# kekeliu-whu/Wildcat-SLAM

Hardware: AMD Instinct MI355X
Metric: surfel-extract Mpts/s (higher is better)
Workload: dtype f64; 1 GPU; C2: 1M-pt single scan (G2 patch lattice, 999936 pts -> 31248 surfels) per GPU, voxel-grid + 3-level octree + per-cell 3x3 PCA; input = the reference's 48-byte hilti_ros::Point records, consumed in place; points_per_gpu=999936, surfels_per_gpu=31248, parallelism=sweep-per-gpu x1

## Files before the change

wildcat-slam_amd/csrc/ctx.h:

```cpp
#pragma once
#include <hip/hip_runtime.h>

#include <cstdarg>
#include <cstdio>
#include <cstdlib>
#include <cstring>
#include <string>
#include <vector>

#include "../../include/wildcat_hip.h"

struct wc_window_state;

struct wc_buf {
  void *p = nullptr;
  size_t cap = 0;
  bool pooled = false;
  bool plain = false;
};

#ifdef WC_DEV_KNOBS
#define WC_DBG(P, bit) ((P).dbg & (bit))
#else
#define WC_DBG(P, bit) 0
#endif

struct wc_dev_opts {
  int exact_sums = 0;
  int debug_skip = 0;
  int fx_merge_min = 3;
  int fx_split = -1;
  int no_bucket_sort = 0;
  int ex_sync = 0;
  int match_pair_serial = 0;
  int lm_dense = 0;
  int lm_side_stream = 1;
  int lm_one_collective = 0;
  int lm_dense_radius = 7;
  int lm_radius0 = -1;
};
inline bool wc_log_env(const char *name) { return getenv(name) != nullptr; }

struct wc_ctx {
  int device = 0;
  wc_params P;
  wc_dev_opts dev;
  bool pool_ok = false;
  hipMemPool_t pool = nullptr;
  hipStream_t own_stream = nullptr;
  hipStream_t stream = nullptr;
  hipEvent_t ev0 = nullptr, ev1 = nullptr;
  std::string err;
  wc_buf b_ex_ctrl;
  wc_buf b_keys[2], b_vals[2], b_sorttmp, b_slots, b_slot_ids, b_slot_keys[2], b_slot_idx[2], b_cand, b_cand_meta,
      b_status, b_misc[8], b_route[4], b_fx[10];
  double match_stats[8] = {0, 0, 0, 0, 0, 0, 0, 0};
  wc_buf b_kd[10];
  std::vector<wc_ctx *> batch_subs;
  wc_buf b_batch;
  wc_buf b_match_half;
  hipEvent_t ev_knn[2] = {nullptr, nullptr};
  wc_comm comm{};
  bool have_comm = false;
  void *rccl = nullptr;
  uint32_t *h_status_dev = nullptr;
  uint32_t *h_status = nullptr;
  unsigned long long mail_ticket = 0;
  wc_buf b_stage;
  void *h_stage = nullptr;
  size_t h_stage_cap = 0;
  double *h_mail = nullptr;
  struct {
    bool active = false;
    wc_points pts;
    double t_lo, t_hi;
    wc_surfel *d_out;
    wc_surfel_id *d_ids;
    uint64_t cap;
    bool wide;
    bool general;
    bool order_general = false;
    int general_calls = 0;
    bool bucket_attr_set = false;
    uint32_t lds_cap = 256;
// ... 101 lines not shown
```

wildcat-slam_amd/csrc/ctx.hip:

```cpp
#include "ctx.h"

#include <cmath>
#include <cstring>
#include <mutex>

extern "C" const char *wc_version(void) { return "wildcat_hip 0.1 (gfx950)"; }

extern "C" int wc_device_count(void) {
  int n = 0;
  if (hipGetDeviceCount(&n) != hipSuccess) return 0;
  return n;
}

extern "C" void wc_params_default(wc_params *p) {
  std::memset(p, 0, sizeof(*p));
  p->voxel_size = 0.8f;
  p->max_layer = 2;
  p->min_points = 20;
  p->planer_threshold = 0.01f;
  p->min_plane_likeness = 0.1;
  p->cluster_gap = 0.05;
  p->cluster_min_points = 20;
  p->center_scale = 1.0;
  p->angular_scale = 5.0 * M_PI / 180.0;
  p->surfel_dist_max = 0.1;
  p->knn_k = 10;
  p->time_diff_min = 0.06;
  p->surfel_sigma0 = 0.05 / 6;
  p->cauchy_a = 0.4;
  const double gn = 0.00015198973532354657, an = 0.006308226052016165;
  const double gw = 0.00011673723527962174, aw = 2.664506559330434e-06;
  const double rate = 200, k = 0.01;
  p->w_gyr = 1 / (gn * std::sqrt(rate)) * k;
  p->w_acc = 1 / (an * std::sqrt(rate)) * k;
  p->w_bg = 1 / (gw / std::sqrt(rate)) * k;
  p->w_ba = 1 / (aw / std::sqrt(rate)) * k;
  p->imu_dt = 1 / rate;
  p->max_iterations = 100;
  p->reference_quirks = 1;
  p->exact_sums = 0;
}

static int check_params(wc_ctx *ctx, const wc_params *p) {
  if (p->max_layer < 0 || p->max_layer > 2) return wc_fail(ctx, WC_ERR_ARG, "max_layer must be 0..2");
  if (!(p->voxel_size > 0)) return wc_fail(ctx, WC_ERR_ARG, "voxel_size must be positive");
  if (p->cluster_min_points < 1 || p->min_points < 0) return wc_fail(ctx, WC_ERR_ARG, "bad point thresholds");
  if (p->knn_k < 1 || p->knn_k > 16) return wc_fail(ctx, WC_ERR_ARG, "knn_k must be 1..16");
  return WC_OK;
}

namespace {
struct DevOpt {
  const char *name, *env;
  int wc_dev_opts::*field;
  bool flag_only;
};
const DevOpt kDevOpts[] = {
    {"exact_sums", "WC_EXACT_SUMS", &wc_dev_opts::exact_sums, true},
    {"debug_skip", "WC_DEBUG_SKIP", &wc_dev_opts::debug_skip, false},
    {"fx_merge_min", "WC_FX_MERGE_MIN", &wc_dev_opts::fx_merge_min, false},
    {"fx_split", "WC_FX_SPLIT", &wc_dev_opts::fx_split, false},
    {"no_bucket_sort", "WC_NO_BUCKET_SORT", &wc_dev_opts::no_bucket_sort, true},
    {"ex_sync", "WC_EX_SYNC", &wc_dev_opts::ex_sync, true},
    {"match_pair_serial", "WC_MATCH_PAIR_SERIAL", &wc_dev_opts::match_pair_serial, true},
    {"lm_dense", "WC_LM_DENSE", &wc_dev_opts::lm_dense, true},
    {"lm_one_collective", "WC_LM_ONE_COLLECTIVE", &wc_dev_opts::lm_one_collective, true},
    {"lm_side_stream", "WC_LM_SIDE_STREAM", &wc_dev_opts::lm_side_stream, false},
    {"lm_dense_radius", "WC_LM_DENSE_RADIUS", &wc_dev_opts::lm_dense_radius, false},
    {"lm_radius0", "WC_LM_RADIUS0", &wc_dev_opts::lm_radius0, false},
};
}

namespace {
struct DevPool {
  hipMemPool_t pool = nullptr;
  int refs = 0;
};
std::mutex g_pool_mu;
DevPool g_pools[64];
}
hipMemPool_t wc_pool_acquire(int device) {
  if (device < 0 || device >= 64) return nullptr;
  std::lock_guard<std::mutex> lk(g_pool_mu);
  DevPool &d = g_pools[device];
  if (!d.pool) {
    int supported = 0;
    if (hipDeviceGetAttribute(&supported, hipDeviceAttributeMemoryPoolsSupported, device) != hipSuccess || !supported) {
      (void)hipGetLastError();
      return nullptr;
    }
    hipMemPoolProps props;
    std::memset(&props, 0, sizeof(props));
    props.allocType = hipMemAllocationTypePinned;
    props.handleTypes = hipMemHandleTypeNone;
    props.location.type = hipMemLocationTypeDevice;
    props.location.id = device;
    hipMemPool_t p = nullptr;
    if (hipMemPoolCreate(&p, &props) != hipSuccess || !p) {
      (void)hipGetLastError();
      return nullptr;
    }
    uint64_t keep = ~0ull;
    if (hipMemPoolSetAttribute(p, hipMemPoolAttrReleaseThreshold, &keep) != hipSuccess) (void)hipGetLastError();
    d.pool = p;
  }
  ++d.refs;
  return d.pool;
}
void wc_pool_release(int device, hipMemPool_t pool) {
  if (!pool || device < 0 || device >= 64) return;
  std::lock_guard<std::mutex> lk(g_pool_mu);
  DevPool &d = g_pools[device];
  if (d.pool == pool && --d.refs == 0) {
    (void)hipMemPoolDestroy(d.pool);
// ... 278 lines not shown
```

wildcat-slam_amd/csrc/extract.hip:

```cpp
#include <hip/hip_runtime.h>
#include <type_traits>

#include <chrono>
#include <cstdlib>
#include <cstring>
#include <rocprim/rocprim.hpp>

#include "ctx.h"
#include "dmath.h"

namespace {

constexpr int kMom = 11;
constexpr int kProdStride = 66;
constexpr unsigned kRootsGrid = 256 * 16;
constexpr unsigned kEmitGrid = 256 * 8;
constexpr unsigned kRoots2Grid = 256 * 4;
constexpr int kBuckets = 4096;
constexpr int kTile = 2048;
constexpr uint32_t kFlagKeyRange = 1u, kFlagSlotOverflow = 2u, kFlagTimeRange = 4u, kFlagBucketOverflow = 8u, kFlagSlotBinOverflow = 16u, kFlagLdsOverflow = 32u;

struct ExParams {
  double vs;
  float vs_f;
// ... 1511 lines not shown
    if (i < nb) {
      s_off[i] = carry + inc - l;
      bin[i] = c;
      run_off[(size_t)b * bin_cap + i] = carry + inc - l;
    }
    carry += __shfl(inc, 63);
  }
  __builtin_amdgcn_wave_barrier();
  uint32_t *s_list = (uint32_t *)s_a;
  uint32_t nlive = 0, next_head = nb;
  for (int i0 = (int)((nb + 63) / 64) * 64 - 64; i0 >= 0; i0 -= 64) {
    const uint32_t r = (uint32_t)i0 + lane;
    const bool in = r < nb;
    const uint32_t rest = in ? comp_rest(s_b[r]) : 0u;
    const bool head = in && (r == 0 || comp_rest(s_b[r - 1]) != rest);
    const unsigned long long hm = __ballot(head);
    const unsigned long long above = (lane == 63) ? 0ull : (hm >> (lane + 1));
    const uint32_t r2 = above ? r + (uint32_t)__ffsll((long long)above) : next_head;
    const uint32_t seg = (r2 < nb ? s_off[min(r2, nb - 1)] : total) - (in ? s_off[r] : 0u);
    const bool live = head && seg > (uint32_t)min_points;
    const unsigned long long lm = __ballot(live);
    if (live) s_list[nlive + (uint32_t)__popcll(lm & ((1ull << lane) - 1ull))] = r | (r2 << 16);
    nlive += (uint32_t)__popcll(lm);
    if (hm) next_head = (uint32_t)i0 + (uint32_t)__ffsll((long long)hm) - 1u;
  }
  if (lane == 0) s_live[w] = nlive;
  __syncthreads();
  const uint32_t pbase0 = s_red[0] + s_red[1] + s_red[2] + s_red[3];
  const uint32_t pbase = pbase0 + before;
  const uint32_t first_slot = pbase0 / (uint32_t)(min_points + 1);
  uint32_t lbase = 0;
  for (int j = 0; j < w; ++j) lbase += s_live[j];
  if (t == 0) {
    root_cnt[blockIdx.x] = s_live[0] + s_live[1] + s_live[2] + s_live[3];
    root_first[blockIdx.x] = first_slot;
  }
  for (uint32_t k = lane; k < nlive; k += 64) {
    const uint32_t r = s_list[k] & 0xFFFFu, r2 = s_list[k] >> 16;
    const uint32_t seg = (r2 < nb ? s_off[r2] : total) - s_off[r];
    head_slots[first_slot + lbase + k] = HeadRec{pbase + s_off[r], b * bin_cap + r, r2 - r, seg};
  }
}

constexpr uint32_t kPtBinMax = 1024;

inline uint32_t pt_bin_cap(uint64_t n) {
  uint32_t cap = 64;
  while (cap < kPtBinMax && (uint64_t)cap * kBuckets < 32 * n) cap *= 2;
  return cap;
}

constexpr uint32_t kCtrlStatus = 0, kCtrlCounts = 64, kCtrlRoots = kCtrlCounts + 2 * kBuckets, kCtrlBins = kCtrlRoots + 2 * (kBuckets / 4),
                   kCtrlFx = kCtrlBins + kBuckets, kCtrlWords = kCtrlFx + 4 * 16 * 32;

int clear_ctrl(wc_ctx *ctx) {
  WC_TRY(wc_ensure(ctx, ctx->b_ex_ctrl, kCtrlWords * 4));
  uint32_t *ctrl = (uint32_t *)ctx->b_ex_ctrl.p;
  InitArgs I{};
  void *dp = nullptr;
  if (hipHostGetDevicePointer(&dp, ctx->h_status, 0) != hipSuccess) dp = nullptr;
  const unsigned long long a = (unsigned long long)dp;
  I.p[0] = ctrl, I.nw[0] = 8, I.val[0] = 0u;
  I.p[1] = ctrl + 10, I.nw[1] = kCtrlRoots - 10, I.val[1] = 0u;
  I.p[2] = ctrl + 8, I.nw[2] = 1, I.val[2] = (uint32_t)a;
  I.p[3] = ctrl + 9, I.nw[3] = 1, I.val[3] = (uint32_t)(a >> 32);
  I.p[4] = ctrl + kCtrlBins, I.nw[4] = kBuckets + 4 * 16 * 32, I.val[4] = 0u;
  k_init<<<(kCtrlRoots + 255) / 256, 256, 0, ctx->stream>>>(I);
  WC_HIP(ctx, hipGetLastError());
  return WC_OK;
}

int point_sort_runs(wc_ctx *ctx, const wc_points &pts, double vs, HeadRec *head_slots, int min_points, uint32_t *status) {
  hipStream_t st = ctx->stream;
  const uint64_t n = pts.n;
  const uint32_t cap = pt_bin_cap(n);
  const uint32_t lds_cap = std::min(cap, std::max(64u, ctx->ex.lds_cap));
  WC_TRY(wc_ensure(ctx, ctx->b_misc[1], (uint64_t)kBuckets * cap * 8));
  WC_TRY(wc_ensure(ctx, ctx->b_misc[3], (uint64_t)kBuckets * cap * 4));
  uint32_t *counts = (uint32_t *)ctx->b_ex_ctrl.p + kCtrlCounts;
  const unsigned tiles = (unsigned)((n + kTile - 1) / kTile);
  const size_t lds = (size_t)4 * lds_cap * 20;
  if (!ctx->ex.bucket_attr_set) {
    WC_HIP(ctx, hipFuncSetAttribute((const void *)k_pt_bucket, hipFuncAttributeMaxDynamicSharedMemorySize, (int)(4 * kPtBinMax * 20)));
    ctx->ex.bucket_attr_set = true;
  }
  k_pt_runs<<<tiles, kRunThreads, 0, st>>>(pts, vs, n, counts, (uint64_t *)ctx->b_misc[1].p, cap, status);
  k_pt_bucket<<<kBuckets / 4, 256, lds, st>>>((uint64_t *)ctx->b_misc[1].p, cap, lds_cap, counts, (uint32_t *)ctx->b_misc[3].p, head_slots,
                                             counts + 2 * kBuckets, counts + 2 * kBuckets + kBuckets / 4, min_points, status);
  WC_HIP(ctx, hipGetLastError());
  return WC_OK;
}

template <typename K>
int sort_pairs(wc_ctx *ctx, K *kin, K *kout, uint32_t *vin, uint32_t *vout, size_t n, unsigned end_bit) {
  using cfg = rocprim::radix_sort_config<rocprim::default_config, rocprim::default_config, rocprim::default_config, 0>;
  size_t tmp = 0;
  WC_HIP(ctx, rocprim::radix_sort_pairs<cfg>(nullptr, tmp, kin, kout, vin, vout, n, 0u, end_bit, ctx->stream));
  WC_TRY(wc_ensure(ctx, ctx->b_sorttmp, tmp));
  tmp = ctx->b_sorttmp.cap;
  WC_HIP(ctx, rocprim::radix_sort_pairs<cfg>(ctx->b_sorttmp.p, tmp, kin, kout, vin, vout, n, 0u, end_bit, ctx->stream));
  return WC_OK;
}

#include "extract_fast.inc"
#include "extract_split.inc"

int fx_ensure_zero(wc_ctx *ctx, wc_buf &b, size_t bytes) {
  if (bytes <= b.cap) return WC_OK;
  WC_TRY(wc_ensure(ctx, b, bytes));
  WC_HIP(ctx, hipMemsetAsync(b.p, 0, b.cap, ctx->stream));
  return WC_OK;
}

bool fx_applicable(const wc_ctx *ctx, uint64_t n, double t_lo, double t_hi) {
  const wc_params &P = ctx->P;
  if (P.exact_sums || ctx->dev.exact_sums) return false;
  if (n < 64 || !(P.voxel_size > 0.0f) || P.voxel_size >= 0.99f) return false;
  if (!(P.cluster_gap > 1e-6) || !(t_hi > t_lo)) return false;
  if ((t_hi - t_lo) / (P.cluster_gap * 0.999) >= 1048000.0) return false;
  return true;
}

int fx_tail(wc_ctx *ctx, bool layer2);

int run_pipeline_fast(wc_ctx *ctx, const wc_points &pts, double t_lo, double t_hi, wc_surfel *d_out, wc_surfel_id *d_ids, uint64_t cap) {
  const wc_params &P = ctx->P;
  const uint64_t n = pts.n;
  hipStream_t st = ctx->stream;
  FxArgs A;
  std::memset(&A, 0, sizeof(A));
  ExParams &E = A.P;
  E.vs = (double)P.voxel_size, E.vs_f = P.voxel_size, E.max_layer = P.max_layer, E.min_points = P.min_points;
  E.thr = (double)P.planer_threshold, E.min_like = P.min_plane_likeness;
  for (int i = 0; i < 3; ++i) E.view[i] = P.view_point[i];
  E.gap = P.cluster_gap, E.cluster_min = P.cluster_min_points;
  E.t_lo_bits = ordered_bits_host(t_lo);
  E.t_span_bits = ordered_bits_host(t_hi) - E.t_lo_bits;
  E.dbg = ctx->dev.debug_skip;
  E.merge_min = ctx->dev.fx_merge_min;
  unsigned tbits = 1;
  while (tbits < 64 && (E.t_span_bits >> tbits)) ++tbits;
  A.pts = pts;
  A.t_lo = t_lo;
  int e = 0;
  (void)std::frexp(t_hi - t_lo, &e);
  A.tick = std::ldexp(1.0, 40 - e), A.inv_tick = std::ldexp(1.0, e - 40);
  A.inv_w = 1.0 / (P.cluster_gap * 0.999);
  A.inv_span = 1.0 / (t_hi - t_lo);
  A.inv_vs = 1.0 / (double)P.voxel_size;
  A.qs = 4294967296.0, A.inv_q = 1.0 / 4294967296.0, A.inv_qq = std::ldexp(1.0, -44);
  uint32_t mr = 1024;
  while ((uint64_t)mr * 8 < n) mr *= 2;
  A.mr_per = mr / kFxSub, A.mq_per = std::max(64u, mr / 2 / kFxSub);
  uint32_t tr = 2048;
  while ((uint64_t)tr * 4 < n) tr *= 2;
  A.tr_mask = tr - 1;
  A.static_map = n <= 2000000ull ? 1u : 0u;
  {
    const uintptr_t px = (uintptr_t)pts.xyz, pt = (uintptr_t)pts.time;
    if (pts.xyz_stride == 48u && pts.time_stride == 48u && pt == px + 24u && px % 16u == 0u)
      A.fmt = 1u;
    else if (pts.xyz_stride == 12u && pts.time_stride == 8u && px % 16u == 0u && pt % 16u == 0u)
      A.fmt = 2u;
  }
  const unsigned tiles = (unsigned)((n + kFxTile - 1) / kFxTile);
  A.rec_tiles = tiles;
  const uint64_t spill_full = ((uint64_t)tiles + 7) / 8 * kFxTile;
  A.spill_per = (uint32_t)((n <= 8000000ull || ctx->ex.fx_spill_full) ? spill_full : std::max<uint64_t>(1024, n / 32));
  A.rec_cap = tiles * (uint32_t)kFxRecTile + 8u * A.spill_per;
  const uint64_t total_slots = std::max<uint64_t>((n * (uint64_t)(P.max_layer + 1)) / (uint64_t)P.cluster_min_points + 1, (uint64_t)kFxSub * 256);
  uint32_t bin_cap = 64;
  while (bin_cap < kSlotBinMax && (uint64_t)bin_cap * kBuckets < 2 * total_slots) bin_cap *= 2;
  WC_TRY(fx_ensure_zero(ctx, ctx->b_fx[0], (size_t)tr * 4));
  WC_TRY(wc_ensure(ctx, ctx->b_fx[1], (size_t)mr * 4));
  WC_TRY(fx_ensure_zero(ctx, ctx->b_fx[2], (size_t)tr * kFxBlockW * 8));
  WC_TRY(fx_ensure_zero(ctx, ctx->b_fx[3], (size_t)A.mq_per * kFxSub * kFxBlockW * 8));
  WC_TRY(wc_ensure(ctx, ctx->b_fx[4], (size_t)2 * A.rec_cap * kFxRecW * 8));
  const unsigned ngrid = std::min<unsigned>(256 * 16, std::max<unsigned>(64, (unsigned)(n / 256)));
  WC_TRY(wc_ensure(ctx, ctx->b_fx[6], (size_t)ngrid * kFxJobCap * kFxJobW * 8));
  ctx->ex.fx_split = ctx->ex.batch_defer || (ctx->dev.fx_split >= 0 ? ctx->dev.fx_split != 0 : !A.static_map);
  if (ctx->ex.fx_split) {
    A.static_map = 0u;
    A.jobpool_per = (uint32_t)std::max<uint64_t>(4096, n / (uint64_t)std::max(1, P.cluster_min_points) / 2);
    WC_TRY(wc_ensure(ctx, ctx->b_fx[7], ((size_t)mr / 8 + 2) * kFxNodeW * 64 * 8));
    WC_TRY(wc_ensure(ctx, ctx->b_fx[8], ((size_t)mr / 8 + 2) * kFxDescW * 4));
    WC_TRY(wc_ensure(ctx, ctx->b_fx[9], (size_t)8 * A.jobpool_per * kFxJobW * 8));
    A.nodes = (unsigned long long *)ctx->b_fx[7].p, A.wdesc = (uint32_t *)ctx->b_fx[8].p, A.jobpool = (unsigned long long *)ctx->b_fx[9].p;
  }
  WC_TRY(wc_ensure(ctx, ctx->b_slots, total_slots * sizeof(wc_surfel)));
  WC_TRY(wc_ensure(ctx, ctx->b_slot_ids, total_slots * sizeof(wc_surfel_id)));
  WC_TRY(wc_ensure(ctx, ctx->b_slot_keys[1], (uint64_t)kBuckets * bin_cap * 8));
  if (ctx->ex.fx_dirty) {
    for (int i : {0, 2, 3}) WC_HIP(ctx, hipMemsetAsync(ctx->b_fx[i].p, 0, ctx->b_fx[i].cap, st));
    ctx->ex.fx_dirty = false;
  }
  WC_TRY(wc_ensure(ctx, ctx->b_fx[5], (size_t)2 * kCtrlWords * 4));
  if (!ctx->ex.fx_ctrl_ready) {
    WC_HIP(ctx, hipMemsetAsync(ctx->b_fx[5].p, 0, (size_t)2 * kCtrlWords * 4, st));
    void *dp = nullptr;
    if (hipHostGetDevicePointer(&dp, ctx->h_status, 0) != hipSuccess) dp = nullptr;
    const unsigned long long a = (unsigned long long)dp;
    const uint32_t addr[2] = {(uint32_t)a, (uint32_t)(a >> 32)};
    for (int b = 0; b < 2; ++b)
      WC_HIP(ctx, hipMemcpyAsync((uint32_t *)ctx->b_fx[5].p + (size_t)b * kCtrlWords + 8, addr, 8, hipMemcpyHostToDevice, st));
    WC_HIP(ctx, hipStreamSynchronize(st));
    ctx->ex.fx_ctrl_ready = true;
    ctx->ex.fx_parity = 0;
  }
  uint32_t *ctrl = (uint32_t *)ctx->b_fx[5].p + (size_t)ctx->ex.fx_parity * kCtrlWords;
  for (int q = 0; q < 64; ++q) ctx->h_status[q] = 0;
// ... 651 lines not shown
```

wildcat-slam_amd/csrc/extract_fast.inc:

```

constexpr uint32_t kFlagFxFallback = 64u;
constexpr int kFxPts = 4;
constexpr int kFxThreads = 256;
constexpr int kFxTile = kFxPts * kFxThreads;
constexpr int kFxLds = 256;
constexpr int kFxLdsProbe = 12;
constexpr int kFxDirect = 16;
constexpr int kFxRecTile = kFxLds + (kFxThreads / 64) * 4 * kFxDirect;
constexpr int kFxSlots = 16;
constexpr int kFxRecW = 16;
constexpr int kFxHdrW = 16;
constexpr int kFxBlockW = kFxHdrW + 8 * kFxSlots / 2;
constexpr int kFxSub = 16;
constexpr uint32_t kFxStRoots = 0, kFxStNodes2 = 1, kFxStSlots = 2, kFxStSpillBank = 3;
constexpr int kFxCntStride = 32;
constexpr int kFxCntWords = 4 * kFxSub * kFxCntStride;
constexpr unsigned long long kFxTMax = 0xFFFFFFFFFFFFull;
constexpr double kFxMagic = 6755399441055744.0, kFxMagic2 = 7083549724304467820544.0;
constexpr unsigned long long kFxMagicBits = 0x4338000000000000ull;
constexpr uint32_t kFxMagicHi = 0x43380000u, kFxMagic2Hi = 0x44780000u;

struct FxArgs {
  wc_points pts;
  ExParams P;
  double t_lo;
  double tick, inv_tick;
  double inv_w;
  double inv_span;
  double inv_vs;
  double qs, inv_q, inv_qq;
  uint32_t *rkey;
  uint32_t *rlist;
  uint32_t tr_mask;
  uint32_t static_map;
  unsigned long long *blk;
  unsigned long long *blk2;
  unsigned long long *rec;
  uint32_t rec_tiles;
  uint32_t spill_per;
  uint32_t rec_cap;
  uint32_t mr_per, mq_per;
  uint32_t fmt;
  uint32_t *status;
  uint32_t *cnt;
  unsigned long long *jobs;
  unsigned long long *nodes;
  uint32_t *wdesc;
  unsigned long long *jobpool;
  uint32_t jobpool_per;
  wc_surfel *slots;
  wc_surfel_id *slot_ids;
  uint32_t slots_per;
  uint32_t *slot_counts;
  uint64_t *slot_bins;
  uint32_t slot_bin_cap;
};

__device__ __forceinline__ void fx_fallback(uint32_t *status, int why) {
  raise_flag(status, kFlagFxFallback);
  uint32_t *hm = host_mailbox(status);
  if (hm) hm[32 + why] = 1u;
}
__device__ __forceinline__ uint32_t *fx_cnt(const FxArgs &A, uint32_t bank, uint32_t j) { return A.cnt + (bank * kFxSub + j) * kFxCntStride; }

__device__ __forceinline__ uint32_t fx_hash32(uint32_t k) {
  k ^= k >> 16;
  k *= 0x7FEB352Du;
  k ^= k >> 15;
  k *= 0x846CA68Bu;
  k ^= k >> 16;
  return k;
}

__device__ __forceinline__ int fx_vox(double p, double vs, double inv_vs) {
  const double q = p * inv_vs;
  const double r = rint(q);
  if (fabs(q - r) > 1e-9 * (fabs(r) + 1.0)) return (int)floor(q);
  return (int)floor(p / vs);
}

constexpr int kFxStMaxProbe = 20;
__device__ __forceinline__ uint32_t fx_root_slot(const FxArgs &A, uint32_t key1, uint32_t sub, bool insert, uint32_t maxprobe = 0u) {
  uint32_t slot = fx_hash32(key1) & A.tr_mask;
  for (int probe = 0; probe < 64; ++probe) {
    uint32_t k;
    if (insert) {
      k = atomicCAS(&A.rkey[slot], 0u, key1);
      if (k == 0u) {
        if (probe) atomicMax(&A.status[kFxStMaxProbe], (uint32_t)probe);
        const uint32_t local = atomicAdd(fx_cnt(A, kFxStRoots, sub), 1u);
        if (local < A.mr_per)
          A.rlist[sub * A.mr_per + local] = slot;
        else
          fx_fallback(A.status, 0);
        return slot;
      }
    } else {
      k = __hip_atomic_load(&A.rkey[slot], __ATOMIC_RELAXED, __HIP_MEMORY_SCOPE_AGENT);
      if (k == 0u && (uint32_t)probe >= maxprobe) return 0xFFFFFFFFu;
    }
    if (k == key1) return slot;
    slot = (slot + 1u) & A.tr_mask;
  }
  fx_fallback(A.status, 1);
  return 0xFFFFFFFFu;
}

struct FxPart {
  uint32_t n;
  long long st, s[3], ss[6];
  unsigned long long tmin_inv, tmax_p1;
};
__device__ __forceinline__ void fx_zero(FxPart &a) {
  a.n = 0, a.st = 0, a.tmin_inv = 0, a.tmax_p1 = 0;
  for (int i = 0; i < 3; ++i) a.s[i] = 0;
  for (int i = 0; i < 6; ++i) a.ss[i] = 0;
}
__device__ __forceinline__ void fx_acc(FxPart &a, const FxPart &b) {
  a.n += b.n, a.st += b.st;
  for (int i = 0; i < 3; ++i) a.s[i] += b.s[i];
  for (int i = 0; i < 6; ++i) a.ss[i] += b.ss[i];
  a.tmin_inv = max(a.tmin_inv, b.tmin_inv);
  a.tmax_p1 = max(a.tmax_p1, b.tmax_p1);
}

__device__ __forceinline__ void fx_add_cell(unsigned long long *cell, const FxPart &a) {
  atomicAdd((uint32_t *)cell, a.n);
  atomicAdd(&cell[1], (unsigned long long)a.st);
  for (int i = 0; i < 3; ++i) atomicAdd(&cell[2 + i], (unsigned long long)a.s[i]);
  for (int i = 0; i < 6; ++i) atomicAdd(&cell[5 + i], (unsigned long long)a.ss[i]);
  atomicMax(&cell[11], a.tmin_inv);
  atomicMax(&cell[12], a.tmax_p1);
}

struct FxEarly {
  uint32_t key1, s0, found;
  int lead;
};
template <int LEVEL>
__device__ __forceinline__ void fx_push(const FxArgs &A, bool active, unsigned long long code, const FxPart &a, uint32_t sub, uint32_t ridx,
                                        const FxEarly &E) {
  const int lane = threadIdx.x & 63;
  unsigned long long *blk = nullptr;
  uint32_t oct, bin, pkey;
  if (LEVEL == 1) {
    pkey = (uint32_t)(code & 0x3FFFFFFFull) + 1u;
    oct = (uint32_t)(code >> 30) & 7u;
    bin = (uint32_t)(code >> 33) & 0xFFFFFu;
  } else {
    pkey = (uint32_t)(code & 0xFFFFFFFull) + 1u;
    oct = (uint32_t)(code >> 28) & 7u;
    bin = (uint32_t)(code >> 31) & 0xFFFFFu;
  }
  int lead = lane;
  uint32_t gmb = bin;
  {
    unsigned long long todo = __ballot(active);
    while (todo) {
      const int first = __ffsll((long long)todo) - 1;
      const uint32_t k0 = (uint32_t)__shfl((int)pkey, first);
      const bool mine = active && pkey == k0;
      uint32_t mb = mine ? bin : 0xFFFFFFFFu;
      for (int m = 1; m < 64; m <<= 1) mb = min(mb, (uint32_t)__shfl_xor((int)mb, m));
      if (mine) lead = first, gmb = mb;
      todo &= ~__ballot(mine);
    }
  }
  const bool leader = active && lane == lead;
  uint32_t slot = 0xFFFFFFFFu;
  bool created = false;
  const uint32_t e_found = (uint32_t)__shfl((int)E.found, E.lead);
  const bool e_have = LEVEL == 1 && E.key1 != 0u && E.key1 == pkey;
  if (leader) {
    if (LEVEL == 1) {
      if (WC_DBG(A.P, 64)) {
        slot = fx_hash32(pkey) & A.tr_mask;
      } else {
        uint32_t s = fx_hash32(pkey) & A.tr_mask;
        int probe = 0;
        if (e_have) {
          if (e_found == 0u || e_found == pkey) {
            slot = s;
          } else {
            s = (s + 1u) & A.tr_mask;
            probe = 1;
          }
        }
        for (; slot == 0xFFFFFFFFu && probe < 64; ++probe) {
          const uint32_t k = atomicCAS(&A.rkey[s], 0u, pkey);
          if (k == 0u || k == pkey) {
            slot = s;
            created = k == 0u;
            if (created && probe) atomicMax(&A.status[kFxStMaxProbe], (uint32_t)probe);
            break;
          }
          s = (s + 1u) & A.tr_mask;
        }
        if (slot == 0xFFFFFFFFu) fx_fallback(A.status, 2);
      }
    } else {
      slot = pkey - 1u;
    }
  }
  const unsigned long long cm = __ballot(created);
  uint32_t list_base = 0;
  const int cfirst = cm ? __ffsll((long long)cm) - 1 : 0;
  if (cm && lane == cfirst) list_base = atomicAdd(fx_cnt(A, kFxStRoots, sub), (uint32_t)__popcll(cm));
  if (leader && slot != 0xFFFFFFFFu && !(WC_DBG(A.P, 8))) {
    unsigned long long *b0 = (LEVEL == 1 ? A.blk : A.blk2) + (size_t)slot * kFxBlockW;
    atomicMax((uint32_t *)b0 + 2, 0xFFFFFFFFu - gmb);
  }
  const uint32_t myslot = (uint32_t)__shfl((int)slot, lead);
  uint32_t old = 0;
  const bool ok = active && myslot != 0xFFFFFFFFu;
  if (ok) {
    blk = (LEVEL == 1 ? A.blk : A.blk2) + (size_t)myslot * kFxBlockW;
    uint32_t *heads = (uint32_t *)(blk + kFxHdrW);
    if (!(WC_DBG(A.P, 32))) old = atomicExch(&heads[oct * kFxSlots + (bin & (kFxSlots - 1))], ridx + 1u);
  }
  if (cm) {
    list_base = (uint32_t)__shfl((int)list_base, cfirst);
    if (created) {
      const uint32_t local = list_base + (uint32_t)__popcll(cm & ((1ull << lane) - 1ull));
      if (local < A.mr_per)
        A.rlist[sub * A.mr_per + local] = slot;
      else
        fx_fallback(A.status, 3);
    }
  }
  if (!ok) return;
  if (WC_DBG(A.P, 16)) return;
  unsigned long long *rec = A.rec + ((size_t)(LEVEL - 1) * A.rec_cap + ridx) * kFxRecW;
  ulonglong2 *r2 = (ulonglong2 *)rec;
  r2[0] = make_ulonglong2((unsigned long long)a.n | ((unsigned long long)bin << 32), (unsigned long long)a.st);
  r2[1] = make_ulonglong2((unsigned long long)a.s[0], (unsigned long long)a.s[1]);
  r2[2] = make_ulonglong2((unsigned long long)a.s[2], (unsigned long long)a.ss[0]);
  r2[3] = make_ulonglong2((unsigned long long)a.ss[1], (unsigned long long)a.ss[2]);
  r2[4] = make_ulonglong2((unsigned long long)a.ss[3], (unsigned long long)a.ss[4]);
  r2[5] = make_ulonglong2((unsigned long long)a.ss[5], a.tmin_inv);
  r2[6] = make_ulonglong2(a.tmax_p1, (unsigned long long)old);
}

struct FxRaw {
  float x[kFxPts], y[kFxPts], z[kFxPts];
  double t[kFxPts];
};
__device__ __forceinline__ FxRaw fx_acc_load(const FxArgs &A, const uint32_t bid) {
  FxRaw r;
  const uint64_t tb = (uint64_t)bid * kFxTile, n = A.pts.n;
#pragma unroll
  for (int it = 0; it < kFxPts; ++it) {
    const uint64_t i = tb + (uint64_t)it * kFxThreads + threadIdx.x;
    r.x[it] = r.y[it] = r.z[it] = 0.f, r.t[it] = 0.0;
    if (i < n) {
      const float *f = (const float *)((const char *)A.pts.xyz + i * A.pts.xyz_stride);
      r.x[it] = f[0], r.y[it] = f[1], r.z[it] = f[2];
      r.t[it] = load_t(A.pts, i);
    }
  }
  return r;
}

template <int LEVEL>
__device__ __forceinline__ void fx_acc_body(const FxArgs &A, const uint32_t bid) {
  __shared__ unsigned long long lds_raw[kFxLds * 14];
  unsigned long long *h_key = lds_raw;
  unsigned long long(*h_rec)[13] = (unsigned long long(*)[13])(lds_raw + kFxLds);
  static_assert(kFxLds * 14 * 8 >= kFxTile * 20, "staging area fits the hash area");
  const int tid = threadIdx.x;
  const ExParams &P = A.P;
  const uint32_t sub = bid & (kFxSub - 1);
  const uint64_t n = A.pts.n;
  const uint64_t base = ((uint64_t)bid * kFxThreads + tid) * kFxPts;
  static_assert(kFxPts == 4, "the LDS transposition reads four points per lane");
  const bool direct = A.fmt == 2u && ((uint64_t)bid + 1u) * kFxTile <= n;
  FxRaw raw;
  float4 da = make_float4(0.f, 0.f, 0.f, 0.f), db = da, dc = da;
  double2 dt01 = make_double2(0.0, 0.0), dt23 = dt01;
  if (direct) {
    const float4 *xp = (const float4 *)((const char *)A.pts.xyz + base * 12u);
    const double2 *tp = (const double2 *)((const char *)A.pts.time + base * 8u);
    da = xp[0], db = xp[1], dc = xp[2];
    dt01 = tp[0], dt23 = tp[1];
  } else {
    raw = fx_acc_load(A, bid);
  }
  double x0, y0, z0;
  load_xyz(A.pts, 0, x0, y0, z0);
  const int k0x = fx_vox(x0, P.vs, A.inv_vs), k0y = fx_vox(y0, P.vs, A.inv_vs), k0z = fx_vox(z0, P.vs, A.inv_vs);
  const float q0 = P.vs_f / 4;

  double px[kFxPts], py[kFxPts], pz[kFxPts], pt[kFxPts];
  if (direct) {
    const float4 a = da, b = db, c = dc;
    const double2 t01 = dt01, t23 = dt23;
    for (int i = tid; i < kFxLds * 14; i += kFxThreads) lds_raw[i] = 0ull;
    px[0] = a.x, py[0] = a.y, pz[0] = a.z, px[1] = a.w, py[1] = b.x, pz[1] = b.y;
    px[2] = b.z, py[2] = b.w, pz[2] = c.x, px[3] = c.y, py[3] = c.z, pz[3] = c.w;
    pt[0] = t01.x, pt[1] = t01.y, pt[2] = t23.x, pt[3] = t23.y;
    __syncthreads();
  } else {
    double *s_t = (double *)lds_raw;
    float *s_x = (float *)(s_t + kFxTile), *s_y = s_x + kFxTile, *s_z = s_y + kFxTile;
#pragma unroll
    for (int it = 0; it < kFxPts; ++it) {
      s_x[it * kFxThreads + tid] = raw.x[it], s_y[it * kFxThreads + tid] = raw.y[it], s_z[it * kFxThreads + tid] = raw.z[it];
      s_t[it * kFxThreads + tid] = raw.t[it];
    }
    __syncthreads();
    {
      const float4 vx = ((const float4 *)s_x)[tid], vy = ((const float4 *)s_y)[tid], vz = ((const float4 *)s_z)[tid];
      const double2 t01 = ((const double2 *)s_t)[2 * tid], t23 = ((const double2 *)s_t)[2 * tid + 1];
      px[0] = vx.x, px[1] = vx.y, px[2] = vx.z, px[3] = vx.w;
      py[0] = vy.x, py[1] = vy.y, py[2] = vy.z, py[3] = vy.w;
      pz[0] = vz.x, pz[1] = vz.y, pz[2] = vz.z, pz[3] = vz.w;
      pt[0] = t01.x, pt[1] = t01.y, pt[2] = t23.x, pt[3] = t23.y;
    }
    __syncthreads();
    for (int i = tid; i < kFxLds * 14; i += kFxThreads) lds_raw[i] = 0ull;
    __syncthreads();
  }
  if (WC_DBG(P, 4)) {
    double sacc = 0;
#pragma unroll
    for (int j = 0; j < kFxPts; ++j) sacc += px[j] + py[j] + pz[j] + pt[j];
    if (sacc == 1.2345) h_key[tid] = 1ull;
    return;
  }
  auto flush_lds = [&](unsigned long long code, const FxPart &a) -> bool {
    uint32_t s = fx_hash32((uint32_t)code ^ (uint32_t)(code >> 29)) & (kFxLds - 1);
    for (int probe = 0; probe < kFxLdsProbe; ++probe) {
      const unsigned long long old = atomicCAS(&h_key[s], 0ull, code);
      if (old == 0ull || old == code) {
        fx_add_cell(&h_rec[s][0], a);
        return true;
      }
      s = (s + 1) & (kFxLds - 1);
    }
    return false;
  };

  unsigned long long code[kFxPts];
  double tmag[kFxPts];
// ... 65 lines not shown
    const double tm = fma(trel, A.tick, kFxMagic);
    const bool time_ok = tm >= kFxMagic && tm < kFxMagic + 2199023255552.0;
    bad_key = bad_key || (have && !key_ok);
    bad_time = bad_time || (have && key_ok && !time_ok);
    bool use = have && key_ok && time_ok;
    const uint32_t bin = (uint32_t)(use ? trel * A.inv_w : 0.0);
    unsigned long long c;
    if (LEVEL == 1) {
      c = (unsigned long long)key | ((unsigned long long)o1 << 30) | ((unsigned long long)bin << 33) | (1ull << 63);
    } else {
      use = use && ((split4[j] >> o1) & 1u);
      const uint32_t qn = base4[j] + (uint32_t)__popc(split4[j] & ((1u << o1) - 1u));
      const double c1x = cx + (double)((float)(2 * bx - 1) * q0), c1y = cy + (double)((float)(2 * by - 1) * q0),
                   c1z = cz + (double)((float)(2 * bz - 1) * q0);
      const uint32_t o2 = (uint32_t)(4 * (x > c1x) + 2 * (y > c1y) + (z > c1z));
      c = (unsigned long long)qn | ((unsigned long long)o2 << 28) | ((unsigned long long)bin << 31) | (1ull << 63);
    }
    const double ccx = cx, ccy = cy, ccz = cz;
    code[j] = use ? c : 0ull;
    tmag[j] = tm;
    const double mx = fma(x - ccx, A.qs, kFxMagic), my = fma(y - ccy, A.qs, kFxMagic), mz = fma(z - ccz, A.qs, kFxMagic);
    qlx[j] = (uint32_t)__double_as_longlong(mx), qly[j] = (uint32_t)__double_as_longlong(my), qlz[j] = (uint32_t)__double_as_longlong(mz);
  }
  if (bad_key) raise_flag(A.status, kFlagKeyRange);
  if (bad_time) raise_flag(A.status, kFlagTimeRange);
  FxEarly early, no_early;
  no_early.key1 = 0u, no_early.s0 = 0u, no_early.found = 0u, no_early.lead = threadIdx.x & 63;
  early = no_early;
  if (LEVEL == 1) {
    unsigned long long lc = 0ull;
#pragma unroll
    for (int j = 0; j < kFxPts; ++j) lc = code[j] ? code[j] : lc;
    const uint32_t pk = lc ? (uint32_t)(lc & 0x3FFFFFFFull) + 1u : 0u;
    unsigned long long todo = __ballot(pk != 0u);
    int lead = threadIdx.x & 63, rounds = 0;
    while (todo && rounds < 4) {
      const int first = __ffsll((long long)todo) - 1;
      const uint32_t k0 = (uint32_t)__shfl((int)pk, first);
      const bool mine = pk != 0u && pk == k0;
      if (mine) lead = first;
      todo &= ~__ballot(mine);
      ++rounds;
    }
    if (!todo && !(WC_DBG(P, 64))) {
      early.key1 = pk;
      early.lead = lead;
      early.s0 = fx_hash32(pk) & A.tr_mask;
      if (pk != 0u && (int)(threadIdx.x & 63) == lead) early.found = atomicCAS(&A.rkey[early.s0], 0u, pk);
    }
  }
  const int lane = tid & 63, wave = tid >> 6;
  const unsigned long long lt_mask = (1ull << lane) - 1ull;
  bool bnd[kFxPts];
  {
    unsigned long long open = 0ull;
#pragma unroll
    for (int j = 0; j < kFxPts; ++j) {
      bnd[j] = code[j] != 0ull && open != 0ull && code[j] != open;
      if (code[j] != 0ull) open = code[j];
    }
  }
  const uint32_t rec0 = bid * (uint32_t)kFxRecTile + (uint32_t)kFxLds + (uint32_t)wave * 4u * (uint32_t)kFxDirect;
  auto close_partial = [&](int cls, bool closing, unsigned long long c, const FxPart &a) {
    const unsigned long long mclass = __ballot(closing);
    if (!mclass || (WC_DBG(P, 2))) return;
    if (__popcll(mclass) <= kFxDirect) {
      fx_push<LEVEL>(A, closing, c & 0x7FFFFFFFFFFFFFFFull, a, sub, rec0 + (uint32_t)cls * (uint32_t)kFxDirect + (uint32_t)__popcll(mclass & lt_mask), cls == 3 ? early : no_early);
    } else {
      const bool failed = closing && !flush_lds(c, a);
      const unsigned long long mf = __ballot(failed);
      if (mf) {
        const uint32_t sp = bid & 7u;
        uint32_t b0 = 0;
        if (lane == 0) b0 = atomicAdd(fx_cnt(A, kFxStSpillBank, sp), (uint32_t)__popcll(mf));
        b0 = (uint32_t)__shfl((int)b0, 0);
        const uint32_t k = b0 + (uint32_t)__popcll(mf & lt_mask);
        const bool room = k < A.spill_per;
        if (failed && !room) fx_fallback(A.status, 4);
        fx_push<LEVEL>(A, failed && room, c & 0x7FFFFFFFFFFFFFFFull, a, sub, A.rec_tiles * (uint32_t)kFxRecTile + sp * A.spill_per + k, no_early);
      }
    }
  };

  FxPart acc;
  double tlo_m = 0.0, thi_m = 0.0;
  uint32_t nfix = 0;
  auto raw_zero = [&]() {
    fx_zero(acc);
    tlo_m = 1.0e300, thi_m = 0.0;
    nfix = 0;
  };
  auto fx_fix = [&]() {
    const uint32_t dn = acc.n - nfix;
    nfix = acc.n;
    const unsigned long long c1 = (unsigned long long)(dn * kFxMagicHi) << 32, c2 = (unsigned long long)(dn * kFxMagic2Hi) << 32;
    acc.st = (long long)((unsigned long long)acc.st - c1);
#pragma unroll
    for (int i = 0; i < 3; ++i) acc.s[i] = (long long)((unsigned long long)acc.s[i] - c1);
#pragma unroll
    for (int i = 0; i < 6; ++i) acc.ss[i] = (long long)((unsigned long long)acc.ss[i] - c2);
    const unsigned long long lo = (unsigned long long)__double_as_longlong(tlo_m) - kFxMagicBits, hi = (unsigned long long)__double_as_longlong(thi_m) - kFxMagicBits;
    acc.tmin_inv = acc.n ? kFxTMax - lo : 0ull;
    acc.tmax_p1 = acc.n ? hi + 1ull : 0ull;
  };
  raw_zero();
  unsigned long long cur = 0ull;
#pragma unroll
  for (int j = 0; j < kFxPts; ++j) {
    if (j) {
      if (__ballot(bnd[j])) {
        fx_fix();
        close_partial(j - 1, bnd[j], cur, acc);
      }
      if (bnd[j]) raw_zero();
    }
    if (code[j] == 0ull) continue;
    cur = code[j];
    acc.n += 1;
    acc.st += __double_as_longlong(tmag[j]);
    const long long bx = (long long)(((unsigned long long)(kFxMagicHi - (qlx[j] >> 31)) << 32) | qlx[j]);
    const long long by = (long long)(((unsigned long long)(kFxMagicHi - (qly[j] >> 31)) << 32) | qly[j]);
    const long long bz = (long long)(((unsigned long long)(kFxMagicHi - (qlz[j] >> 31)) << 32) | qlz[j]);
    acc.s[0] += bx, acc.s[1] += by, acc.s[2] += bz;
    const double x = __longlong_as_double(bx) - kFxMagic, y = __longlong_as_double(by) - kFxMagic, z = __longlong_as_double(bz) - kFxMagic;
    acc.ss[0] += __double_as_longlong(fma(x, x, kFxMagic2)), acc.ss[1] += __double_as_longlong(fma(x, y, kFxMagic2));
    acc.ss[2] += __double_as_longlong(fma(x, z, kFxMagic2)), acc.ss[3] += __double_as_longlong(fma(y, y, kFxMagic2));
    acc.ss[4] += __double_as_longlong(fma(y, z, kFxMagic2)), acc.ss[5] += __double_as_longlong(fma(z, z, kFxMagic2));
    tlo_m = fmin(tlo_m, tmag[j]), thi_m = fmax(thi_m, tmag[j]);
  }
  fx_fix();
  bool e_made = false;
  unsigned long long e_cm = 0ull;
  uint32_t e_base = 0;
  if (LEVEL == 1) {
    e_made = early.key1 != 0u && (int)(threadIdx.x & 63) == early.lead && early.found == 0u;
    e_cm = __ballot(e_made);
    if (e_cm && (int)(threadIdx.x & 63) == __ffsll((long long)e_cm) - 1) e_base = atomicAdd(fx_cnt(A, kFxStRoots, sub), (uint32_t)__popcll(e_cm));
  }
  {
    const unsigned long long mycode = acc.n ? cur : 0ull;
    auto shr32 = [](uint32_t v, auto dtag) -> uint32_t {
      constexpr int d = decltype(dtag)::value;
      return (uint32_t)__builtin_amdgcn_update_dpp(0, (int)v, 0x110 + d, 0xF, 0xF, true);
    };
    auto shr64 = [&](unsigned long long v, auto dtag) -> unsigned long long {
      return (unsigned long long)shr32((uint32_t)v, dtag) | ((unsigned long long)shr32((uint32_t)(v >> 32), dtag) << 32);
    };
    const int rl = lane & 15;
    const unsigned long long prevc = shr64(mycode, std::integral_constant<int, 1>{});
    uint32_t head = (rl == 0 || prevc != mycode) ? 1u : 0u;
    auto step = [&](auto dtag) {
      constexpr int d = decltype(dtag)::value;
      if (!__ballot(rl >= d && !head)) return;
      const uint32_t ohead = shr32(head, dtag);
      const uint32_t on = shr32(acc.n, dtag);
      const long long ost = (long long)shr64((unsigned long long)acc.st, dtag);
      long long os[3], oss[6];
#pragma unroll
      for (int i = 0; i < 3; ++i) os[i] = (long long)shr64((unsigned long long)acc.s[i], dtag);
#pragma unroll
      for (int i = 0; i < 6; ++i) oss[i] = (long long)shr64((unsigned long long)acc.ss[i], dtag);
      const unsigned long long omin = shr64(acc.tmin_inv, dtag), omax = shr64(acc.tmax_p1, dtag);
      if (rl >= d && !head) {
        acc.n += on, acc.st += ost;
#pragma unroll
        for (int i = 0; i < 3; ++i) acc.s[i] += os[i];
#pragma unroll
        for (int i = 0; i < 6; ++i) acc.ss[i] += oss[i];
        acc.tmin_inv = max(acc.tmin_inv, omin);
        acc.tmax_p1 = max(acc.tmax_p1, omax);
        head = ohead;
      }
    };
    step(std::integral_constant<int, 1>{});
    step(std::integral_constant<int, 2>{});
    step(std::integral_constant<int, 4>{});
    step(std::integral_constant<int, 8>{});
    const uint32_t nlo = (uint32_t)__builtin_amdgcn_update_dpp(0, (int)(uint32_t)mycode, 0x101, 0xF, 0xF, true);
    const uint32_t nhi = (uint32_t)__builtin_amdgcn_update_dpp(0, (int)(uint32_t)(mycode >> 32), 0x101, 0xF, 0xF, true);
    const unsigned long long nextc = (unsigned long long)nlo | ((unsigned long long)nhi << 32);
    const bool tail = mycode != 0ull && (rl == 15 || nextc != mycode);
    close_partial(3, tail, mycode, acc);
  }
  __syncthreads();
  if (WC_DBG(P, 1)) return;
  static_assert(kFxLds == kFxThreads, "one hash cell per thread in the final loop");
  {
    const int i = tid;
    const unsigned long long c = h_key[i];
    FxPart a;
    fx_zero(a);
    if (c != 0ull) {
      a.n = (uint32_t)h_rec[i][0];
      a.st = (long long)h_rec[i][1];
      for (int w = 0; w < 3; ++w) a.s[w] = (long long)h_rec[i][2 + w];
      for (int w = 0; w < 6; ++w) a.ss[w] = (long long)h_rec[i][5 + w];
      a.tmin_inv = h_rec[i][11];
      a.tmax_p1 = h_rec[i][12];
    }
    if (__ballot(c != 0ull)) fx_push<LEVEL>(A, c != 0ull, c & 0x7FFFFFFFFFFFFFFFull, a, sub, bid * (uint32_t)kFxRecTile + (uint32_t)i, no_early);
  }
  if (LEVEL == 1 && e_cm) {
    const int l = threadIdx.x & 63;
    const uint32_t list_base = (uint32_t)__shfl((int)e_base, __ffsll((long long)e_cm) - 1);
    if (e_made) {
      const uint32_t local = list_base + (uint32_t)__popcll(e_cm & ((1ull << l) - 1ull));
      if (local < A.mr_per)
        A.rlist[sub * A.mr_per + local] = early.s0;
      else
        fx_fallback(A.status, 5);
    }
  }
}

template <int LEVEL>
__global__ void __launch_bounds__(kFxThreads) k_fx_acc(FxArgs A) {
  fx_acc_body<LEVEL>(A, blockIdx.x);
}

struct FxBatch {
  const FxArgs *args;
  const uint32_t *start;
  const uint32_t *flags;
  int K;
};
__device__ __forceinline__ int fx_batch_find(const FxBatch &B, uint32_t b, uint32_t &local) {
  int k = 0;
  while (k + 1 < B.K && b >= B.start[k + 1]) ++k;
  local = b - B.start[k];
  return k;
}
#define WC_FX_BATCH_ARGS(sA, B, k)                                                                 \
  __shared__ FxArgs sA;                                                                            \
  static_assert(sizeof(FxArgs) % 8 == 0, "copied as 64-bit words");                                 \
// ... 670 lines not shown
      }
      if ((split >> gl) & 1u) {
        const uint32_t qn = first + (uint32_t)__popc(split & ((1u << gl) - 1u));
        uint32_t *q32 = (uint32_t *)(A.blk2 + (size_t)qn * kFxBlockW);
        const bool first_child = (split & ((1u << gl) - 1u)) == 0u;
        q32[0] = pidx | ((uint32_t)gl << 28) | (first_child ? 0x80000000u : 0u);
        q32[1] = key + 1u;
      }
    }
  }
  return queued;
}

__device__ __forceinline__ void fx_clear_heads(unsigned long long *blk) {
  uint4 *hz = (uint4 *)(blk + kFxHdrW) + (threadIdx.x & 7) * 4;
  hz[0] = hz[1] = hz[2] = hz[3] = make_uint4(0u, 0u, 0u, 0u);
}
template <int LEVEL>
__device__ __forceinline__ void fx_clear_header(const FxArgs &A, unsigned long long *blk, uint32_t pidx, bool queued) {
  uint32_t *w32 = (uint32_t *)blk;
  if (LEVEL == 1) {
    if (!queued) {
      w32[2] = 0u;
      A.rkey[pidx] = 0u;
    }
  } else {
    const uint32_t ro = w32[0];
    w32[0] = w32[1] = w32[2] = 0u;
    if (ro & 0x80000000u) {
      const uint32_t rslot = ro & 0xFFFFFFFu;
      uint32_t *r32 = (uint32_t *)(A.blk + (size_t)rslot * kFxBlockW);
      r32[2] = r32[12] = r32[13] = 0u;
      A.rkey[rslot] = 0u;
    }
  }
}

constexpr FxWhy kFxWhyNodes = {7, 8, 9, 10, 11, 12, -1};
template <int LEVEL>
__global__ void __launch_bounds__(64) k_fx_nodes(FxArgs A) {
  __shared__ uint32_t s_heads[64][kFxSlots + 1];
  __shared__ unsigned long long s_root[8][kFxSlots][13];
  __shared__ uint8_t s_jown[kFxJobCap];
  __shared__ uint8_t s_flag[72];
  __shared__ uint32_t s_gkey[8], s_go1p[8];
  const ExParams &P = A.P;
  const int lane = threadIdx.x, g = lane >> 3, gl = lane & 7;
  const uint32_t bank = LEVEL == 1 ? kFxStRoots : kFxStNodes2;
  const uint32_t per = LEVEL == 1 ? A.mr_per : A.mq_per;
  const bool stat = A.static_map != 0u;
  const uint32_t sj = blockIdx.x & (kFxSub - 1);
  const uint32_t nwj = (gridDim.x - sj + kFxSub - 1) / kFxSub;
  uint32_t total = 0, cnts[kFxSub], cnt_j = 0;
  if (stat) {
    cnt_j = min(*fx_cnt(A, bank, (int)sj), per);
  } else {
#pragma unroll
    for (int j = 0; j < kFxSub; ++j) {
      cnts[j] = min(*fx_cnt(A, bank, j), per);
      total += cnts[j];
    }
  }
  double x0, y0, z0;
  load_xyz(A.pts, 0, x0, y0, z0);
  const int k0x = vox(x0, P.vs), k0y = vox(y0, P.vs), k0z = vox(z0, P.vs);
  const float q0 = P.vs_f / 4;
  const uint32_t wsub = blockIdx.x & (kFxSub - 1);
  if (WC_DBG(P, 2048)) return;
  for (uint32_t it = 0;; ++it) {
    uint32_t pidx = 0;
    bool have_parent;
    if (stat) {
      const uint32_t chunk = blockIdx.x / kFxSub + it * nwj;
      if (chunk * 8u >= per) break;
      const uint32_t local = chunk * 8u + (uint32_t)g;
      pidx = sj * per + min(local, per - 1u);
      if (LEVEL == 1) {
        pidx = A.rlist[pidx] & A.tr_mask;
        asm volatile("" : "+v"(pidx));
      }
      if (chunk * 8u >= cnt_j) break;
      have_parent = local < cnt_j;
    } else {
      const uint32_t w0 = (blockIdx.x + it * gridDim.x) * 8u;
      if (w0 >= total) break;
      const uint32_t gi = w0 + (uint32_t)g;
      have_parent = gi < total;
      pidx = fx_dense_parent<LEVEL>(A, cnts, per, gi, have_parent);
    }
    unsigned long long *blk = (LEVEL == 1 ? A.blk : A.blk2) + (size_t)pidx * kFxBlockW;
    uint32_t key, o1p, minbin;
    fx_parent_header<LEVEL>(A, blk, pidx, have_parent, key, o1p, minbin);
    int kx, ky, kz;
    double cc[3];
    fx_key_voxel(P, key, k0x, k0y, k0z, kx, ky, kz, cc);
    const uint32_t occ = fx_load_heads(blk, have_parent, minbin, s_heads[lane]);
    uint32_t jcnt = 0;
    const bool one_bin = __ballot((occ & (occ - 1u)) != 0u) == 0ull;
    if (LEVEL == 1 && !one_bin) {
      for (int i = lane; i < 8 * kFxSlots * 13; i += 64) (&s_root[0][0][0])[i] = 0ull;
      __builtin_amdgcn_wave_barrier();
    }
    unsigned long long *jb = A.jobs + (size_t)blockIdx.x * kFxJobCap * kFxJobW;
    auto push_job = [&](bool closing, const FxPart &cl, uint32_t ordv, uint32_t owner) {
      const uint32_t pos = fx_push_job(A, jb, jcnt, closing, cl, ordv, owner, kFxWhyNodes.jobs);
      if (pos < (uint32_t)kFxJobCap) s_jown[pos] = (uint8_t)owner;
    };
    FxPart tot;
    uint32_t ncl;
    fx_walk_node<LEVEL, kFxChains>(A, occ, minbin, s_heads[lane], LEVEL == 1 && !one_bin, s_root[g], kFxWhyNodes, push_job, tot, ncl);
    __builtin_amdgcn_wave_barrier();
    FxPart rt;
    bool parent_live;
    uint32_t split;
    const FxEmit pend = fx_test_children<LEVEL>(A, have_parent, tot, ncl, key, o1p, kx, ky, kz, cc, q0, wsub, kFxWhyNodes.slots, s_flag, s_gkey, s_go1p,
                                                rt, parent_live, split);
    if (LEVEL == 1) {
      fx_test_root(A, parent_live, rt, cc, kx, ky, kz, q0, wsub, kFxWhyNodes.slots, s_flag, [&](bool rpl) -> uint32_t {
// ... 43 lines not shown
```

Before: 21530 Mpts/s.

## Issue fast-path hash link atomics early and pass voxel origin via counter line

Splits the per-segment push into a link step (atomic slot claim and chain head exchange) and a store step. The link atomics for each closing class are issued before accumulation so their latency overlaps with the sum computation; the record stores follow later. Separately, the level-1 kernel writes the first point's voxel coordinates next to the sub-counters, and k_fx_nodes reads count and origin with one 16-byte load instead of reloading and re-voxelizing the point. This holds l_ok/l_old state in registers across the accumulation loop, adding register pressure, and it is gated by a new dev option that defaults to on.

```diff
diff --git a/wildcat-slam_amd/csrc/ctx.h b/wildcat-slam_amd/csrc/ctx.h
--- a/wildcat-slam_amd/csrc/ctx.h
+++ b/wildcat-slam_amd/csrc/ctx.h
@@ -30,6 +30,7 @@
   int debug_skip = 0;
   int fx_merge_min = 3;
   int fx_split = -1;
+  int fx_early_link = 1;
   int no_bucket_sort = 0;
   int ex_sync = 0;
   int match_pair_serial = 0;
diff --git a/wildcat-slam_amd/csrc/ctx.hip b/wildcat-slam_amd/csrc/ctx.hip
--- a/wildcat-slam_amd/csrc/ctx.hip
+++ b/wildcat-slam_amd/csrc/ctx.hip
@@ -60,6 +60,7 @@
     {"debug_skip", "WC_DEBUG_SKIP", &wc_dev_opts::debug_skip, false},
     {"fx_merge_min", "WC_FX_MERGE_MIN", &wc_dev_opts::fx_merge_min, false},
     {"fx_split", "WC_FX_SPLIT", &wc_dev_opts::fx_split, false},
+    {"fx_early_link", "WC_FX_EARLY_LINK", &wc_dev_opts::fx_early_link, false},
     {"no_bucket_sort", "WC_NO_BUCKET_SORT", &wc_dev_opts::no_bucket_sort, true},
     {"ex_sync", "WC_EX_SYNC", &wc_dev_opts::ex_sync, true},
     {"match_pair_serial", "WC_MATCH_PAIR_SERIAL", &wc_dev_opts::match_pair_serial, true},
diff --git a/wildcat-slam_amd/csrc/extract.hip b/wildcat-slam_amd/csrc/extract.hip
--- a/wildcat-slam_amd/csrc/extract.hip
+++ b/wildcat-slam_amd/csrc/extract.hip
@@ -1587,6 +1587,7 @@
 
 constexpr uint32_t kCtrlStatus = 0, kCtrlCounts = 64, kCtrlRoots = kCtrlCounts + 2 * kBuckets, kCtrlBins = kCtrlRoots + 2 * (kBuckets / 4),
                    kCtrlFx = kCtrlBins + kBuckets, kCtrlWords = kCtrlFx + 4 * 16 * 32;
+static_assert(kCtrlFx % 32 == 0 && kCtrlWords % 32 == 0, "every sub-counter of the fast path starts a 128-byte line (k_fx_nodes reads 16 bytes of it)");
 
 int clear_ctrl(wc_ctx *ctx) {
   WC_TRY(wc_ensure(ctx, ctx->b_ex_ctrl, kCtrlWords * 4));
@@ -1691,6 +1692,7 @@
   while ((uint64_t)tr * 4 < n) tr *= 2;
   A.tr_mask = tr - 1;
   A.static_map = n <= 2000000ull ? 1u : 0u;
+  A.early_link = ctx->dev.fx_early_link != 0 ? 1u : 0u;
   {
     const uintptr_t px = (uintptr_t)pts.xyz, pt = (uintptr_t)pts.time;
     if (pts.xyz_stride == 48u && pts.time_stride == 48u && pt == px + 24u && px % 16u == 0u)
diff --git a/wildcat-slam_amd/csrc/extract_fast.inc b/wildcat-slam_amd/csrc/extract_fast.inc
--- a/wildcat-slam_amd/csrc/extract_fast.inc
+++ b/wildcat-slam_amd/csrc/extract_fast.inc
@@ -33,6 +33,7 @@
   uint32_t *rlist;
   uint32_t tr_mask;
   uint32_t static_map;
+  uint32_t early_link;
   unsigned long long *blk;
   unsigned long long *blk2;
   unsigned long long *rec;
@@ -138,8 +139,8 @@
   int lead;
 };
 template <int LEVEL>
-__device__ __forceinline__ void fx_push(const FxArgs &A, bool active, unsigned long long code, const FxPart &a, uint32_t sub, uint32_t ridx,
-                                        const FxEarly &E) {
+__device__ __forceinline__ void fx_push_link(const FxArgs &A, bool active, unsigned long long code, uint32_t sub, uint32_t ridx, const FxEarly &E,
+                                             bool &ok_out, uint32_t &old_out) {
   const int lane = threadIdx.x & 63;
   unsigned long long *blk = nullptr;
   uint32_t oct, bin, pkey;
@@ -228,8 +229,13 @@
         fx_fallback(A.status, 3);
     }
   }
+  ok_out = ok, old_out = old;
+}
+template <int LEVEL>
+__device__ __forceinline__ void fx_push_store(const FxArgs &A, bool ok, unsigned long long code, const FxPart &a, uint32_t ridx, uint32_t old) {
   if (!ok) return;
   if (WC_DBG(A.P, 16)) return;
+  const uint32_t bin = (uint32_t)(code >> (LEVEL == 1 ? 33 : 31)) & 0xFFFFFu;
   unsigned long long *rec = A.rec + ((size_t)(LEVEL - 1) * A.rec_cap + ridx) * kFxRecW;
   ulonglong2 *r2 = (ulonglong2 *)rec;
   r2[0] = make_ulonglong2((unsigned long long)a.n | ((unsigned long long)bin << 32), (unsigned long long)a.st);
@@ -239,6 +245,14 @@
   r2[4] = make_ulonglong2((unsigned long long)a.ss[3], (unsigned long long)a.ss[4]);
   r2[5] = make_ulonglong2((unsigned long long)a.ss[5], a.tmin_inv);
   r2[6] = make_ulonglong2(a.tmax_p1, (unsigned long long)old);
+}
+template <int LEVEL>
+__device__ __forceinline__ void fx_push(const FxArgs &A, bool active, unsigned long long code, const FxPart &a, uint32_t sub, uint32_t ridx,
+                                        const FxEarly &E) {
+  bool ok;
+  uint32_t old;
+  fx_push_link<LEVEL>(A, active, code, sub, ridx, E, ok, old);
+  fx_push_store<LEVEL>(A, ok, code, a, ridx, old);
 }
 
 struct FxRaw {
@@ -289,6 +303,10 @@
   load_xyz(A.pts, 0, x0, y0, z0);
   const int k0x = fx_vox(x0, P.vs, A.inv_vs), k0y = fx_vox(y0, P.vs, A.inv_vs), k0z = fx_vox(z0, P.vs, A.inv_vs);
   const float q0 = P.vs_f / 4;
+  if (LEVEL == 1 && bid == 0u && tid < 2 * kFxSub) {
+    uint32_t *c = fx_cnt(A, tid < kFxSub ? kFxStRoots : kFxStNodes2, (uint32_t)tid & (kFxSub - 1));
+    c[1] = (uint32_t)k0x, c[2] = (uint32_t)k0y, c[3] = (uint32_t)k0z;
+  }
 
   double px[kFxPts], py[kFxPts], pz[kFxPts], pt[kFxPts];
   if (direct) {
@@ -460,20 +478,45 @@
   const int lane = tid & 63, wave = tid >> 6;
   const unsigned long long lt_mask = (1ull << lane) - 1ull;
   bool bnd[kFxPts];
+  unsigned long long pcode[kFxPts];
+  unsigned long long mycode = 0ull;
   {
-    unsigned long long open = 0ull;
 #pragma unroll
     for (int j = 0; j < kFxPts; ++j) {
-      bnd[j] = code[j] != 0ull && open != 0ull && code[j] != open;
-      if (code[j] != 0ull) open = code[j];
-    }
+      pcode[j] = mycode;
+      bnd[j] = code[j] != 0ull && mycode != 0ull && code[j] != mycode;
+      if (code[j] != 0ull) mycode = code[j];
+    }
+  }
+  bool tail;
+  {
+    const uint32_t nlo = (uint32_t)__builtin_amdgcn_update_dpp(0, (int)(uint32_t)mycode, 0x101, 0xF, 0xF, true);
+    const uint32_t nhi = (uint32_t)__builtin_amdgcn_update_dpp(0, (int)(uint32_t)(mycode >> 32), 0x101, 0xF, 0xF, true);
+    const unsigned long long nextc = (unsigned long long)nlo | ((unsigned long long)nhi << 32);
+    tail = mycode != 0ull && ((lane & 15) == 15 || nextc != mycode);
   }
   const uint32_t rec0 = bid * (uint32_t)kFxRecTile + (uint32_t)kFxLds + (uint32_t)wave * 4u * (uint32_t)kFxDirect;
+  uint32_t linked = 0u;
+  bool l_ok[4] = {false, false, false, false};
+  uint32_t l_old[4] = {0u, 0u, 0u, 0u};
+  auto link_class = [&](int cls, bool closing, unsigned long long c) {
+    const unsigned long long mclass = __ballot(closing);
+    if (!A.early_link || !mclass || (WC_DBG(P, 2)) || __popcll(mclass) > kFxDirect) return;
+    linked |= 1u << cls;
+    fx_push_link<LEVEL>(A, closing, c & 0x7FFFFFFFFFFFFFFFull, sub, rec0 + (uint32_t)cls * (uint32_t)kFxDirect + (uint32_t)__popcll(mclass & lt_mask),
+                        cls == 3 ? early : no_early, l_ok[cls], l_old[cls]);
+  };
+#pragma unroll
+  for (int j = 1; j < kFxPts; ++j) link_class(j - 1, bnd[j], pcode[j]);
+  link_class(3, tail, mycode);
   auto close_partial = [&](int cls, bool closing, unsigned long long c, const FxPart &a) {
     const unsigned long long mclass = __ballot(closing);
     if (!mclass || (WC_DBG(P, 2))) return;
-    if (__popcll(mclass) <= kFxDirect) {
-      fx_push<LEVEL>(A, closing, c & 0x7FFFFFFFFFFFFFFFull, a, sub, rec0 + (uint32_t)cls * (uint32_t)kFxDirect + (uint32_t)__popcll(mclass & lt_mask), cls == 3 ? early : no_early);
+    const uint32_t ridx = rec0 + (uint32_t)cls * (uint32_t)kFxDirect + (uint32_t)__popcll(mclass & lt_mask);
+    if ((linked >> cls) & 1u) {
+      fx_push_store<LEVEL>(A, l_ok[cls], c & 0x7FFFFFFFFFFFFFFFull, a, ridx, l_old[cls]);
+    } else if (__popcll(mclass) <= kFxDirect) {
+      fx_push<LEVEL>(A, closing, c & 0x7FFFFFFFFFFFFFFFull, a, sub, ridx, cls == 3 ? early : no_early);
     } else {
       const bool failed = closing && !flush_lds(c, a);
       const unsigned long long mf = __ballot(failed);
@@ -512,18 +555,16 @@
     acc.tmax_p1 = acc.n ? hi + 1ull : 0ull;
   };
   raw_zero();
-  unsigned long long cur = 0ull;
 #pragma unroll
   for (int j = 0; j < kFxPts; ++j) {
     if (j) {
       if (__ballot(bnd[j])) {
         fx_fix();
-        close_partial(j - 1, bnd[j], cur, acc);
+        close_partial(j - 1, bnd[j], pcode[j], acc);
       }
       if (bnd[j]) raw_zero();
     }
     if (code[j] == 0ull) continue;
-    cur = code[j];
     acc.n += 1;
     acc.st += __double_as_longlong(tmag[j]);
     const long long bx = (long long)(((unsigned long long)(kFxMagicHi - (qlx[j] >> 31)) << 32) | qlx[j]);
@@ -546,7 +587,6 @@
     if (e_cm && (int)(threadIdx.x & 63) == __ffsll((long long)e_cm) - 1) e_base = atomicAdd(fx_cnt(A, kFxStRoots, sub), (uint32_t)__popcll(e_cm));
   }
   {
-    const unsigned long long mycode = acc.n ? cur : 0ull;
     auto shr32 = [](uint32_t v, auto dtag) -> uint32_t {
       constexpr int d = decltype(dtag)::value;
       return (uint32_t)__builtin_amdgcn_update_dpp(0, (int)v, 0x110 + d, 0xF, 0xF, true);
@@ -584,10 +624,6 @@
     step(std::integral_constant<int, 2>{});
     step(std::integral_constant<int, 4>{});
     step(std::integral_constant<int, 8>{});
-    const uint32_t nlo = (uint32_t)__builtin_amdgcn_update_dpp(0, (int)(uint32_t)mycode, 0x101, 0xF, 0xF, true);
-    const uint32_t nhi = (uint32_t)__builtin_amdgcn_update_dpp(0, (int)(uint32_t)(mycode >> 32), 0x101, 0xF, 0xF, true);
-    const unsigned long long nextc = (unsigned long long)nlo | ((unsigned long long)nhi << 32);
-    const bool tail = mycode != 0ull && (rl == 15 || nextc != mycode);
     close_partial(3, tail, mycode, acc);
   }
   __syncthreads();
@@ -1364,8 +1400,9 @@
   const uint32_t sj = blockIdx.x & (kFxSub - 1);
   const uint32_t nwj = (gridDim.x - sj + kFxSub - 1) / kFxSub;
   uint32_t total = 0, cnts[kFxSub], cnt_j = 0;
+  const uint4 c4 = *(const uint4 *)fx_cnt(A, bank, stat ? sj : 0u);
   if (stat) {
-    cnt_j = min(*fx_cnt(A, bank, (int)sj), per);
+    cnt_j = min(c4.x, per);
   } else {
 #pragma unroll
     for (int j = 0; j < kFxSub; ++j) {
@@ -1373,9 +1410,7 @@
       total += cnts[j];
     }
   }
-  double x0, y0, z0;
-  load_xyz(A.pts, 0, x0, y0, z0);
-  const int k0x = vox(x0, P.vs), k0y = vox(y0, P.vs), k0z = vox(z0, P.vs);
+  const int k0x = (int)c4.y, k0y = (int)c4.z, k0z = (int)c4.w;
   const float q0 = P.vs_f / 4;
   const uint32_t wsub = blockIdx.x & (kFxSub - 1);
   if (WC_DBG(P, 2048)) return;
```

New measurement: 22020 Mpts/s (median of 4 runs). 1.02x the previous value.
